# Ced3-han/PepFlowww

Hardware: AMD Instinct MI355X
Metric: residues x denoise-steps / s (higher is better)
Workload: dtype f32 (fp32 storage and accumulation; matrix products as 3 x f16 split MFMA, ~22-bit operands); 1 GPU; cfg4/GPU: B=64 x 128-residue synthetic pockets (112 ctx + 16 gen) per GPU; per_gpu_batch=64, residues=128, global_batch=64, parallelism=batch-shard x1, hipgraph=True, precision=fp32

## Files before the change

pepflowww_amd/csrc/node_track.hip:

```cpp
#include "common.h"
#include "rigid_dev.h"
#include "../../include/pepflow_hip.h"

#ifdef PF_PROFILE
__device__ long long g_prof[64];
#ifndef PF_PROF_LAST
#define PF_PROF_LAST 1
#endif
#define PROF(i) do { if (LAST == (PF_PROF_LAST != 0) && blockIdx.x == 0 && threadIdx.x == 0) g_prof[i] = clock64(); } while (0)
extern "C" int pf_debug_prof(long long* out, int n) {
    return (int)hipMemcpyFromSymbol(out, HIP_SYMBOL(g_prof), sizeof(long long) * n, 0, hipMemcpyDeviceToHost);
}
#else
#define PROF(i)
#endif

namespace {

constexpr int TR = 16;
constexpr int LDX = 132;
constexpr int LDP = 136;
constexpr int NTHR = 512;
#ifndef PF_NT_MINW
#define PF_NT_MINW 2
#endif

struct Planes { _Float16* h; _Float16* l; };

struct LnParams { float g[8], b[8]; };
__device__ __forceinline__ void ln_load(LnParams& p, const float* __restrict__ g, const float* __restrict__ b) {
    const int sub = threadIdx.x & 15;
    const float4 g0 = *reinterpret_cast<const float4*>(g + 8 * sub), g1 = *reinterpret_cast<const float4*>(g + 8 * sub + 4);
    const float4 b0 = *reinterpret_cast<const float4*>(b + 8 * sub), b1 = *reinterpret_cast<const float4*>(b + 8 * sub + 4);
    p.g[0] = g0.x; p.g[1] = g0.y; p.g[2] = g0.z; p.g[3] = g0.w; p.g[4] = g1.x; p.g[5] = g1.y; p.g[6] = g1.z; p.g[7] = g1.w;
    p.b[0] = b0.x; p.b[1] = b0.y; p.b[2] = b0.z; p.b[3] = b0.w; p.b[4] = b1.x; p.b[5] = b1.y; p.b[6] = b1.z; p.b[7] = b1.w;
}
template <int ROWS = 16, bool KFR = false>
__device__ __forceinline__ void ln_tile(float* T, const LnParams& p, float mk, Planes out, int m0, int M, float* gout, _Float16* kf = nullptr, int i0 = 0) {
    const int tid = threadIdx.x;
    if (tid < 16 * ROWS) {
        const int row = tid >> 4, sub = tid & 15, m = m0 + row;
        float v[8];
        {
            const float4 a = *reinterpret_cast<const float4*>(T + row * LDX + 8 * sub);
            const float4 b = *reinterpret_cast<const float4*>(T + row * LDX + 8 * sub + 4);
            v[0] = a.x; v[1] = a.y; v[2] = a.z; v[3] = a.w; v[4] = b.x; v[5] = b.y; v[6] = b.z; v[7] = b.w;
        }
        float s = ((v[0] + v[1]) + (v[2] + v[3])) + ((v[4] + v[5]) + (v[6] + v[7]));
        s = row16_sum(s);
        const float mean = s / 128.f;
        float q = 0.f;
#pragma unroll
        for (int c = 0; c < 8; ++c) { const float d = v[c] - mean; q += d * d; }
        q = row16_sum(q);
        const float rstd = rsqrtf(q / 128.f + 1e-5f);
        float y[8];
#pragma unroll
        for (int c = 0; c < 8; ++c) y[c] = ((v[c] - mean) * rstd * p.g[c] + p.b[c]) * mk;
        *reinterpret_cast<float4*>(T + row * LDX + 8 * sub) = make_float4(y[0], y[1], y[2], y[3]);
        *reinterpret_cast<float4*>(T + row * LDX + 8 * sub + 4) = make_float4(y[4], y[5], y[6], y[7]);
        half4 h0, l0, h1, l1;
        const float y0[4] = {y[0], y[1], y[2], y[3]}, y1[4] = {y[4], y[5], y[6], y[7]};
        split4(y0, h0, l0);
        split4(y1, h1, l1);
        *reinterpret_cast<half4*>(out.h + row * LDP + 8 * sub) = h0;
        *reinterpret_cast<half4*>(out.h + row * LDP + 8 * sub + 4) = h1;
        *reinterpret_cast<half4*>(out.l + row * LDP + 8 * sub) = l0;
        *reinterpret_cast<half4*>(out.l + row * LDP + 8 * sub + 4) = l1;
        if (gout && m < M) {
            *reinterpret_cast<float4*>(gout + (size_t)m * 128 + 8 * sub) = make_float4(y[0], y[1], y[2], y[3]);
            *reinterpret_cast<float4*>(gout + (size_t)m * 128 + 8 * sub + 4) = make_float4(y[4], y[5], y[6], y[7]);
        }
        if constexpr (KFR) {
            if (kf && m < M) {
                pf_kfrag_put(kf, i0 + row, sub >> 1, 2 * (sub & 1), y0);
                pf_kfrag_put(kf, i0 + row, sub >> 1, 2 * (sub & 1) + 1, y1);
            }
        }
    }
}

__device__ __forceinline__ float4 sel4(bool ok, const float4& v) {
    const float f = ok ? 1.f : 0.f;
    return make_float4(v.x * f, v.y * f, v.z * f, v.w * f);
}

__device__ __forceinline__ void put_planes(Planes p, int r, int n, const float (&v)[4]) {
    half4 hi, lo;
    split4(v, hi, lo);
    *reinterpret_cast<half4*>(p.h + r * LDP + n) = hi;
    *reinterpret_cast<half4*>(p.l + r * LDP + n) = lo;
}

template <bool SP, bool DUMP = false, bool PM = false>
__global__ __launch_bounds__(NTHR, PF_NT_MINW) void node_head_kernel(pf_node_head_args a) {
    extern __shared__ __attribute__((aligned(16))) unsigned char smem_raw[];
    constexpr int CK = 256, LDC = CK + 8;
    _Float16* Ch = reinterpret_cast<_Float16*>(smem_raw);
    float* X = reinterpret_cast<float*>(smem_raw + 2 * 2 * TR * LDC * sizeof(_Float16));
    Planes Xa = {reinterpret_cast<_Float16*>(X + TR * LDX), reinterpret_cast<_Float16*>(X + TR * LDX) + TR * LDP};
    const int tid = threadIdx.x, wave = tid >> 6, lane = tid & 63;
    const int r = lane & 15, g = lane >> 4;
    const int m0 = blockIdx.x * TR, M = a.rows;
    if (pf_rows_all_masked(a.key_end, a.key_L, m0, TR, M)) return;
    const int n = wave * 16 + 4 * g;

    constexpr int C0 = PM ? 4 : 0;
    WSplit<1, 8, SP> ws;
    ws.init(a.w_out_f16, 128, PF_IPA_FEATS - C0 * 256, wave * 16);
    ws.prefetch();
    LnParams lnp;
    ln_load(lnp, a.ln_g, a.ln_b);
    const float4 bias_out = *reinterpret_cast<const float4*>(a.b_out + n);
    float4 bias_in[3];
#pragma unroll
    for (int wt = 0; wt < 3; ++wt) bias_in[wt] = *reinterpret_cast<const float4*>(a.b_in + wave * 48 + wt * 16 + 4 * g);
    const int mr = m0 + r;
    const int mrc = mr < M ? mr : M - 1;
    const float rmask_ld = a.mask[mrc];
    const float4 rres_ld = *reinterpret_cast<const float4*>(a.s_in + (size_t)mrc * 128 + n);
    const int srow = tid >> 5, sc4 = tid & 31;
    const bool sok = m0 + srow < M;
    const float* src = a.feats + (size_t)(sok ? m0 + srow : 0) * PF_IPA_FEATS + 4 * sc4;
    constexpr int NCH = PF_IPA_FEATS / CK;
    float4 st[NCH][2];
#pragma unroll
    for (int c = 0; c < NCH; ++c)
#pragma unroll
        for (int hlf = 0; hlf < 2; ++hlf)
            st[c][hlf] = *reinterpret_cast<const float4*>(src + c * CK + hlf * 128);
    auto commit = [&](int c) {
        _Float16* bh = Ch + (c & 1) * 2 * TR * LDC;
        _Float16* bl = bh + TR * LDC;
#pragma unroll
        for (int hlf = 0; hlf < 2; ++hlf) {
            const float4 sv = sel4(sok, st[c][hlf]);
            const float v[4] = {sv.x, sv.y, sv.z, sv.w};
            half4 hi, lo;
            split4(v, hi, lo);
            *reinterpret_cast<half4*>(bh + srow * LDC + hlf * 128 + 4 * sc4) = hi;
            *reinterpret_cast<half4*>(bl + srow * LDC + hlf * 128 + 4 * sc4) = lo;
        }
    };
    if constexpr (PM) {
        auto add4 = [](const float4& p, const float4& q) { return make_float4(p.x + q.x, p.y + q.y, p.z + q.z, p.w + q.w); };
        float4 ev = sel4(sok, st[0][0]), od = sel4(sok, st[0][1]);
#pragma unroll
        for (int c = 1; c < 4; ++c) { ev = add4(ev, sel4(sok, st[c][0])); od = add4(od, sel4(sok, st[c][1])); }
        *reinterpret_cast<float4*>(X + srow * LDX + 4 * sc4) = add4(ev, od);
    }
    commit(C0);
    __syncthreads();
    f32x4 am[1], ac[1];
    acc_zero1<1>(am, ac);
#pragma unroll
    for (int c = C0; c < NCH; ++c) {
        const _Float16* bh = Ch + (c & 1) * 2 * TR * LDC;
        gemm_split16(ws, bh, bh + TR * LDC, LDC, am, ac, (c - C0) * 8, 8);
        if (c + 1 < NCH) commit(c + 1);
        __syncthreads();
    }
    WSplit<3, 4, SP> wq;
    wq.init(a.w_in_f16, 384, 128, wave * 48);
    wq.prefetch();
    {
        const float rmask = rmask_ld * (mr < M ? 1.f : 0.f);
        const float4 rres = sel4(mr < M, rres_ld);
        float4 hs = make_float4(0.f, 0.f, 0.f, 0.f);
        if constexpr (PM) hs = *reinterpret_cast<const float4*>(X + r * LDX + n);
        auto lin = [&](int e, float h) { const float j = join(am[0], ac[0], e); if constexpr (PM) return j + h; else return j; };
        float4 y;
        y.x = (lin(0, hs.x) + bias_out.x) * rmask + rres.x;
        y.y = (lin(1, hs.y) + bias_out.y) * rmask + rres.y;
        y.z = (lin(2, hs.z) + bias_out.z) * rmask + rres.z;
        y.w = (lin(3, hs.w) + bias_out.w) * rmask + rres.w;
        *reinterpret_cast<float4*>(X + r * LDX + n) = y;
        if constexpr (DUMP) { if (mr < M) *reinterpret_cast<float4*>(a.dump_a0 + (size_t)mr * 128 + n) = y; }
    }
    __syncthreads();
    ln_tile(X, lnp, 1.f, Xa, m0, M, a.s_ipa);
    __syncthreads();
    f32x4 qm[3], qc[3];
    acc_zero1<3>(qm, qc);
    gemm_split16(wq, Xa.h, Xa.l, LDP, qm, qc, 0, 4);
    if (mr < M) {
#pragma unroll
        for (int wt = 0; wt < 3; ++wt) {
            float4 y;
            y.x = join(qm[wt], qc[wt], 0) + bias_in[wt].x; y.y = join(qm[wt], qc[wt], 1) + bias_in[wt].y;
            y.z = join(qm[wt], qc[wt], 2) + bias_in[wt].z; y.w = join(qm[wt], qc[wt], 3) + bias_in[wt].w;
            *reinterpret_cast<float4*>(a.qkv + (size_t)mr * 384 + wave * 48 + wt * 16 + 4 * g) = y;
        }
    }
}

constexpr int TR2 = 32;
template <bool SP, bool PM = false>
__global__ __launch_bounds__(NTHR, PF_NT_MINW) void node_head32_kernel(pf_node_head_args a) {
    extern __shared__ __attribute__((aligned(16))) unsigned char smem_raw[];
    constexpr int CK = 256, LDC = CK + 8;
    _Float16* Ch = reinterpret_cast<_Float16*>(smem_raw);
    float* X = reinterpret_cast<float*>(smem_raw + 2 * 2 * TR2 * LDC * sizeof(_Float16));
    Planes Xa = {reinterpret_cast<_Float16*>(X + TR2 * LDX), reinterpret_cast<_Float16*>(X + TR2 * LDX) + TR2 * LDP};
    const int tid = threadIdx.x, wave = tid >> 6, lane = tid & 63;
    const int r = lane & 15, g = lane >> 4;
    int m0 = blockIdx.x * TR2, M = a.rows;
    if (a.key_end) {
        const int tps = (a.key_L + TR2 - 1) / TR2, b = blockIdx.x / tps, i0 = (blockIdx.x - b * tps) * TR2;
        if (i0 >= a.key_end[b]) return;
        m0 = b * a.key_L + i0;
        M = (b + 1) * a.key_L;
    }
    const int n = wave * 16 + 4 * g;

    constexpr int C0 = PM ? 4 : 0;
    WSplit<1, 8, SP> ws;
    ws.init(a.w_out_f16, 128, PF_IPA_FEATS - C0 * 256, wave * 16);
    ws.prefetch();
    LnParams lnp;
    ln_load(lnp, a.ln_g, a.ln_b);
    const float4 bias_out = *reinterpret_cast<const float4*>(a.b_out + n);
    float4 bias_in[3];
#pragma unroll
    for (int wt = 0; wt < 3; ++wt) bias_in[wt] = *reinterpret_cast<const float4*>(a.b_in + wave * 48 + wt * 16 + 4 * g);
    float rmask_ld[2];
    float4 rres_ld[2];
#pragma unroll
    for (int rt = 0; rt < 2; ++rt) {
        const int mr = m0 + rt * 16 + r;
        const int mrc = mr < M ? mr : M - 1;
        rmask_ld[rt] = a.mask[mrc];
        rres_ld[rt] = *reinterpret_cast<const float4*>(a.s_in + (size_t)mrc * 128 + n);
    }
    constexpr int NCH = PF_IPA_FEATS / CK;
    float4 st[2][4];
    auto fetch = [&](int c, float4 (&d)[4]) {
#pragma unroll
        for (int u = 0; u < 4; ++u) {
            const int idx = tid + u * NTHR, row = idx >> 6, c4 = idx & 63;
            const int m = m0 + row < M ? m0 + row : M - 1;
            d[u] = *reinterpret_cast<const float4*>(a.feats + (size_t)m * PF_IPA_FEATS + c * CK + 4 * c4);
        }
    };
    auto commit = [&](int c, const float4 (&d)[4]) {
        _Float16* bh = Ch + (c & 1) * 2 * TR2 * LDC;
        _Float16* bl = bh + TR2 * LDC;
#pragma unroll
        for (int u = 0; u < 4; ++u) {
            const int idx = tid + u * NTHR, row = idx >> 6, c4 = idx & 63;
            const float4 sv = sel4(m0 + row < M, d[u]);
            const float v[4] = {sv.x, sv.y, sv.z, sv.w};
            half4 hi, lo;
            split4(v, hi, lo);
            *reinterpret_cast<half4*>(bh + row * LDC + 4 * c4) = hi;
            *reinterpret_cast<half4*>(bl + row * LDC + 4 * c4) = lo;
        }
    };
    fetch(0, st[0]);
    fetch(1, st[1]);
    if constexpr (PM) {
        auto add4 = [](const float4& p, const float4& q) { return make_float4(p.x + q.x, p.y + q.y, p.z + q.z, p.w + q.w); };
        float4 hsum[4];
#pragma unroll
        for (int c = 0; c < 4; ++c) {
#pragma unroll
            for (int u = 0; u < 4; ++u) {
                const int idx = tid + u * NTHR, row = idx >> 6;
                const float4 v = sel4(m0 + row < M, st[c & 1][u]);
                hsum[u] = c == 0 ? v : add4(hsum[u], v);
            }
            fetch(c + 2, st[c & 1]);
        }
#pragma unroll
        for (int u = 0; u < 4; ++u) {
            const int idx = tid + u * NTHR, row = idx >> 6, c4 = idx & 63;
            float4 o;
            o.x = __shfl_xor(hsum[u].x, 32); o.y = __shfl_xor(hsum[u].y, 32); o.z = __shfl_xor(hsum[u].z, 32); o.w = __shfl_xor(hsum[u].w, 32);
            if (c4 < 32) *reinterpret_cast<float4*>(X + row * LDX + 4 * c4) = add4(hsum[u], o);
        }
    }
    commit(C0, st[C0 & 1]);
    __syncthreads();
    f32x4 am[2][1], ac[2][1];
#pragma unroll
    for (int rt = 0; rt < 2; ++rt) acc_zero1<1>(am[rt], ac[rt]);
#pragma unroll
    for (int c = C0; c < NCH; ++c) {
        if (!PM && c + 2 < NCH) fetch(c + 2, st[c & 1]);
        const _Float16* bh = Ch + (c & 1) * 2 * TR2 * LDC;
        gemm_split16r<1, 8, SP, 2>(ws, bh, bh + TR2 * LDC, LDC, am, ac, (c - C0) * 8, 8);
        if (c + 1 < NCH) commit(c + 1, st[(c + 1) & 1]);
        __syncthreads();
    }
    WSplit<3, 4, SP> wq;
    wq.init(a.w_in_f16, 384, 128, wave * 48);
    wq.prefetch();
#pragma unroll
    for (int rt = 0; rt < 2; ++rt) {
        const int mr = m0 + rt * 16 + r;
        const float rmask = rmask_ld[rt] * (mr < M ? 1.f : 0.f);
        const float4 rres = sel4(mr < M, rres_ld[rt]);
        float4 hs = make_float4(0.f, 0.f, 0.f, 0.f);
        if constexpr (PM) hs = *reinterpret_cast<const float4*>(X + (rt * 16 + r) * LDX + n);
        auto lin = [&](int e, float h) { const float j = join(am[rt][0], ac[rt][0], e); if constexpr (PM) return j + h; else return j; };
        float4 y;
        y.x = (lin(0, hs.x) + bias_out.x) * rmask + rres.x;
        y.y = (lin(1, hs.y) + bias_out.y) * rmask + rres.y;
        y.z = (lin(2, hs.z) + bias_out.z) * rmask + rres.z;
        y.w = (lin(3, hs.w) + bias_out.w) * rmask + rres.w;
        *reinterpret_cast<float4*>(X + (rt * 16 + r) * LDX + n) = y;
    }
    __syncthreads();
    ln_tile<TR2>(X, lnp, 1.f, Xa, m0, M, a.s_ipa);
    __syncthreads();
    f32x4 qm[2][3], qc[2][3];
#pragma unroll
    for (int rt = 0; rt < 2; ++rt) acc_zero1<3>(qm[rt], qc[rt]);
    gemm_split16r<3, 4, SP, 2>(wq, Xa.h, Xa.l, LDP, qm, qc, 0, 4);
#pragma unroll
    for (int rt = 0; rt < 2; ++rt) {
        const int mr = m0 + rt * 16 + r;
        if (mr < M) {
#pragma unroll
            for (int wt = 0; wt < 3; ++wt) {
                float4 y;
                y.x = join(qm[rt][wt], qc[rt][wt], 0) + bias_in[wt].x; y.y = join(qm[rt][wt], qc[rt][wt], 1) + bias_in[wt].y;
                y.z = join(qm[rt][wt], qc[rt][wt], 2) + bias_in[wt].z; y.w = join(qm[rt][wt], qc[rt][wt], 3) + bias_in[wt].w;
                *reinterpret_cast<float4*>(a.qkv + (size_t)mr * 384 + wave * 48 + wt * 16 + 4 * g) = y;
            }
        }
    }
}

template <bool LAST, bool SP, int RT, bool DUMP = false>
__global__ __launch_bounds__(NTHR, PF_NT_MINW) void node_tfmr_kernel(pf_node_tfmr_args a, int LP, int LDS_S) {
    constexpr int TR = 16 * RT;
    extern __shared__ __attribute__((aligned(16))) float smem[];
    float* T0 = smem;
    float* T1 = T0 + TR * LDX;
    float* U = T1 + TR * LDX;
    _Float16* pl = reinterpret_cast<_Float16*>(U + TR * 8);
    Planes Xa = {pl, pl + TR * LDP}, Xb = {pl + 2 * TR * LDP, pl + 3 * TR * LDP};
    float* S = reinterpret_cast<float*>(pl + 4 * TR * LDP);
    const int tid = threadIdx.x, wave = tid >> 6, lane = tid & 63;
    const int r = lane & 15, g = lane >> 4;
    const int L = a.L;
    const int tiles = (L + TR - 1) / TR;
    const int lid = a.key_end ? (int)blockIdx.x : xcd_remap(blockIdx.x, gridDim.x);
    const int b = lid / tiles;
    const int i0 = (lid - b * tiles) * TR;
    const size_t rowb = (size_t)b * L;
    if (a.key_end && i0 >= __builtin_amdgcn_readfirstlane(a.key_end[b])) return;
    if constexpr (LAST) {
        if (a.row_on) {
            int any = 0;
#pragma unroll
            for (int rt = 0; rt < RT; ++rt) any |= a.row_on[((int)rowb + min(i0 + 16 * rt, L - 16)) >> 4];
            if (!__builtin_amdgcn_readfirstlane(any)) return;
        }
    }
    const int m0 = (int)rowb + i0;
    const int M = (int)rowb + L;
    const int n = wave * 16 + 4 * g;
    int mr[RT];
#pragma unroll
    for (int rt = 0; rt < RT; ++rt) mr[rt] = m0 + 16 * rt + r;
    auto dump4 = [&](float* p, int rt, float x, float y, float z, float w) {
        if constexpr (DUMP) { if (mr[rt] < M) *reinterpret_cast<float4*>(p + (size_t)mr[rt] * 128 + n) = make_float4(x, y, z, w); }
    };

    PROF(0);
    const int h = wave & 3;
    float4 q0[RT], q1[RT];
#pragma unroll
    for (int rt = 0; rt < RT; ++rt) {
        const int i = i0 + 16 * rt + r;
        const float* qrow = a.qkv + (rowb + (i < L ? i : 0)) * 384 + h * 32 + 4 * g;
        q0[rt] = *reinterpret_cast<const float4*>(qrow);
        q1[rt] = *reinterpret_cast<const float4*>(qrow + 16);
    }
    const float4 z4 = make_float4(0.f, 0.f, 0.f, 0.f);
    const int par = wave >> 2;
    auto kload = [&](int j0, float4 (&k0)[2], float4 (&k1)[2], float (&km)[2]) {
#pragma unroll
        for (int t = 0; t < 2; ++t) {
            const int j = j0 + 32 * t + r;
            const int jc = j < L ? j : L - 1;
            const float* krow = a.qkv + (rowb + jc) * 384 + 128 + h * 32 + 4 * g;
            k0[t] = *reinterpret_cast<const float4*>(krow);
            k1[t] = *reinterpret_cast<const float4*>(krow + 16);
            km[t] = a.mask[rowb + jc];
        }
    };
    float4 kfA0[2], kfA1[2], kfB0[2], kfB1[2];
    float kfAm[2], kfBm[2];
    kload(16 * par, kfA0, kfA1, kfAm);
    kload(16 * par + 64, kfB0, kfB1, kfBm);
    asm volatile("" ::: "memory");
    const int ct = wave >> 2;
    const float* vcol = a.qkv + rowb * 384 + 256 + h * 32 + ct * 16 + r;
    auto vload = [&](int k0, float (&vb)[4][4]) {
#pragma unroll
        for (int s4 = 0; s4 < 4; ++s4)
#pragma unroll
            for (int t = 0; t < 4; ++t) {
                int j = k0 + 16 * s4 + 4 * g + t;
                j = j < L ? j : L - 1;
                vb[s4][t] = vcol[(size_t)j * 384];
            }
    };
    float vbA[4][4], vbB[4][4];
    vload(0, vbA);
    vload(64, vbB);
    asm volatile("" ::: "memory");
    WSplit<1, 4, SP> ws;
    ws.init(a.w_o_f16, 128, 128, wave * 16);
    ws.prefetch();
    LnParams ln1, ln2, ln3;
    ln_load(ln1, a.n1_g, a.n1_b);
    ln_load(ln2, a.n2_g, a.n2_b);
    if (LAST) ln_load(ln3, a.nt_g, a.nt_b);
    const float4 bias_o = *reinterpret_cast<const float4*>(a.b_o + n), bias_1 = *reinterpret_cast<const float4*>(a.b_1 + n),
                 bias_2 = *reinterpret_cast<const float4*>(a.b_2 + n);
    float4 bias_post = z4, bias_t1 = z4, bias_t2 = z4, bias_t3 = z4, bias_bb = z4, bias_init = z4;
    float4 bias_in[3] = {z4, z4, z4}, bias_pre[4] = {z4, z4, z4, z4};
    float4 rres_ld[RT], rsipa_ld[RT];
#pragma unroll
    for (int rt = 0; rt < RT; ++rt) {
        const int mrc = mr[rt] < M ? mr[rt] : M - 1;
        rres_ld[rt] = *reinterpret_cast<const float4*>(a.resid + (size_t)mrc * 128 + n);
        rsipa_ld[rt] = LAST ? *reinterpret_cast<const float4*>(a.s_ipa + (size_t)mrc * 128 + n) : z4;
    }
    float lnmask_ld = 1.f;
    const int lnrow = m0 + ((tid & (16 * TR - 1)) >> 4);
    auto load_tail_consts = [&]() {
        bias_post = *reinterpret_cast<const float4*>(a.b_post + n);
        bias_t1 = *reinterpret_cast<const float4*>(a.b_t1 + n);
        bias_t2 = *reinterpret_cast<const float4*>(a.b_t2 + n);
        bias_t3 = *reinterpret_cast<const float4*>(a.b_t3 + n);
        bias_bb = *reinterpret_cast<const float4*>(a.b_bb + 4 * (g & 1));
        if (a.has_et) {
            bias_init = *reinterpret_cast<const float4*>(a.b_init + (wave & 3) * 16 + 4 * g);
#pragma unroll
            for (int wt = 0; wt < 4; ++wt) bias_pre[wt] = *reinterpret_cast<const float4*>(a.b_pre + wave * 64 + wt * 16 + 4 * g);
        }
        lnmask_ld = a.mask[lnrow < M ? lnrow : M - 1];
    };
    if (LAST) {
        if (RT == 1) load_tail_consts();
    } else {
#pragma unroll
        for (int wt = 0; wt < 3; ++wt) bias_in[wt] = *reinterpret_cast<const float4*>(a.b_in_next + wave * 48 + wt * 16 + 4 * g);
    }

    PROF(1);
    {
        const float scale = 0.17677669529663687f;
        auto score_block = [&](int j0, const float4 (&k0)[2], const float4 (&k1)[2], const float (&km)[2]) {
#pragma unroll
            for (int t = 0; t < 2; ++t) {
                const int j = j0 + 32 * t + r;
                if (j0 + 32 * t < LP) {
                    const bool keep = j < L && km[t] > 0.5f;
#pragma unroll
                    for (int rt = 0; rt < RT; ++rt) {
                        f32x4 acc = {0.f, 0.f, 0.f, 0.f};
                        acc = mfma16(q0[rt].x, k0[t].x, acc); acc = mfma16(q0[rt].y, k0[t].y, acc); acc = mfma16(q0[rt].z, k0[t].z, acc); acc = mfma16(q0[rt].w, k0[t].w, acc);
                        acc = mfma16(q1[rt].x, k1[t].x, acc); acc = mfma16(q1[rt].y, k1[t].y, acc); acc = mfma16(q1[rt].z, k1[t].z, acc); acc = mfma16(q1[rt].w, k1[t].w, acc);
#pragma unroll
                        for (int e = 0; e < 4; ++e) S[((16 * rt + 4 * g + e) * 4 + h) * LDS_S + j] = keep ? acc[e] * scale : -3.0e38f;
                    }
                }
            }
        };
        score_block(16 * par, kfA0, kfA1, kfAm);
        if (16 * par + 64 < LP) score_block(16 * par + 64, kfB0, kfB1, kfBm);
        for (int j0 = 16 * par + 128; j0 < LP; j0 += 64) {
            float4 kn0[2], kn1[2];
            float knm[2];
            kload(j0, kn0, kn1, knm);
            score_block(j0, kn0, kn1, knm);
        }
    }
    __syncthreads();
    PROF(2);
#pragma unroll
    for (int ps = 0; ps < RT; ++ps) {
        const int sub = lane & 7;
        float* sp = S + ((ps * 8 + wave) * 8 + (lane >> 3)) * LDS_S;
        if (LP <= 256) {
            float4 v[8];
#pragma unroll
            for (int u = 0; u < 8; ++u) {
                const int j = 4 * sub + 32 * u;
                v[u] = j < LP ? *reinterpret_cast<const float4*>(sp + j) : make_float4(-3.0e38f, -3.0e38f, -3.0e38f, -3.0e38f);
            }
            float m = -3.0e38f;
#pragma unroll
            for (int u = 0; u < 8; ++u) m = fmaxf(m, fmaxf(fmaxf(v[u].x, v[u].y), fmaxf(v[u].z, v[u].w)));
            m = fmaxf(m, lane_xor1(m)); m = fmaxf(m, lane_xor2(m)); m = fmaxf(m, lane_xor4(m));
            float sum = 0.f;
#pragma unroll
            for (int u = 0; u < 8; ++u) {
                v[u].x = (v[u].x > -1.0e38f) ? exp_softmax(v[u].x - m) : 0.f; v[u].y = (v[u].y > -1.0e38f) ? exp_softmax(v[u].y - m) : 0.f;
                v[u].z = (v[u].z > -1.0e38f) ? exp_softmax(v[u].z - m) : 0.f; v[u].w = (v[u].w > -1.0e38f) ? exp_softmax(v[u].w - m) : 0.f;
                sum += (v[u].x + v[u].y) + (v[u].z + v[u].w);
            }
            sum += lane_xor1(sum); sum += lane_xor2(sum); sum += lane_xor4(sum);
            const float inv = 1.f / sum;
#pragma unroll
            for (int u = 0; u < 8; ++u) {
                const int j = 4 * sub + 32 * u;
                if (j < LP) *reinterpret_cast<float4*>(sp + j) = make_float4(v[u].x * inv, v[u].y * inv, v[u].z * inv, v[u].w * inv);
            }
        } else {
            float m = -3.0e38f;
            for (int j = sub; j < LP; j += 8) m = fmaxf(m, sp[j]);
            m = fmaxf(m, lane_xor1(m)); m = fmaxf(m, lane_xor2(m)); m = fmaxf(m, lane_xor4(m));
            float sum = 0.f;
            for (int j = sub; j < LP; j += 8) { const float e = (sp[j] > -1.0e38f) ? exp_softmax(sp[j] - m) : 0.f; sp[j] = e; sum += e; }
            sum += lane_xor1(sum); sum += lane_xor2(sum); sum += lane_xor4(sum);
            const float inv = 1.f / sum;
            for (int j = sub; j < LP; j += 8) sp[j] *= inv;
        }
    }
    __syncthreads();
    PROF(3);
    {
        f32x4 acc[RT];
#pragma unroll
        for (int rt = 0; rt < RT; ++rt) acc[rt] = (f32x4){0.f, 0.f, 0.f, 0.f};
        const float* prow = S + (r * 4 + h) * LDS_S + 4 * g;
        auto pv_block = [&](int k0, const float (&vb)[4][4]) {
#pragma unroll
            for (int s4 = 0; s4 < 4; ++s4) {
                if (k0 + 16 * s4 < LP) {
#pragma unroll
                    for (int rt = 0; rt < RT; ++rt) {
                        const float4 pa = *reinterpret_cast<const float4*>(prow + rt * 64 * LDS_S + k0 + 16 * s4);
                        acc[rt] = mfma16(pa.x, vb[s4][0], acc[rt]); acc[rt] = mfma16(pa.y, vb[s4][1], acc[rt]);
                        acc[rt] = mfma16(pa.z, vb[s4][2], acc[rt]); acc[rt] = mfma16(pa.w, vb[s4][3], acc[rt]);
                    }
                }
            }
        };
        pv_block(0, vbA);
        if (64 < LP) pv_block(64, vbB);
        for (int k0 = 128; k0 < LP; k0 += 64) {
            float vn[4][4];
            vload(k0, vn);
            pv_block(k0, vn);
        }
        const int col = h * 32 + ct * 16 + r;
#pragma unroll
        for (int rt = 0; rt < RT; ++rt)
#pragma unroll
            for (int e = 0; e < 4; ++e) {
                const _Float16 hi = (_Float16)acc[rt][e];
                Xa.h[(16 * rt + 4 * g + e) * LDP + col] = hi;
                Xa.l[(16 * rt + 4 * g + e) * LDP + col] = (_Float16)((acc[rt][e] - (float)hi) * PF_LO_SCALE);
                if constexpr (DUMP) { if (m0 + 16 * rt + 4 * g + e < M) a.dump[0][(size_t)(m0 + 16 * rt + 4 * g + e) * 128 + col] = acc[rt][e]; }
            }
    }
    if (LAST && RT == 2) load_tail_consts();
    __syncthreads();
    PROF(4);

    f32x4 am[RT][1], ac[RT][1];
    auto zero = [&]() {
#pragma unroll
        for (int rt = 0; rt < RT; ++rt) acc_zero1<1>(am[rt], ac[rt]);
    };
    auto joined = [&](int rt, const float4& bias, float (&v)[4]) {
        v[0] = join(am[rt][0], ac[rt][0], 0) + bias.x; v[1] = join(am[rt][0], ac[rt][0], 1) + bias.y;
        v[2] = join(am[rt][0], ac[rt][0], 2) + bias.z; v[3] = join(am[rt][0], ac[rt][0], 3) + bias.w;
    };
    auto relu4 = [](float (&v)[4]) {
#pragma unroll
        for (int e = 0; e < 4; ++e) v[e] = fmaxf(v[e], 0.f);
    };
    zero();
    gemm_split16r<1, 4, SP, RT>(ws, Xa.h, Xa.l, LDP, am, ac, 0, 4);
    ws.init(a.w_1_f16, 128, 128, wave * 16);
    ws.prefetch();
#pragma unroll
    for (int rt = 0; rt < RT; ++rt) {
        const float4 rres = sel4(mr[rt] < M, rres_ld[rt]);
        float v[4];
        joined(rt, bias_o, v);
        *reinterpret_cast<float4*>(T1 + (16 * rt + r) * LDX + n) = make_float4(v[0] + rres.x, v[1] + rres.y, v[2] + rres.z, v[3] + rres.w);
        dump4(a.dump[1], rt, v[0] + rres.x, v[1] + rres.y, v[2] + rres.z, v[3] + rres.w);
    }
    __syncthreads();
    ln_tile<TR>(T1, ln1, 1.f, Xb, m0, M, DUMP ? a.dump[2] : nullptr);
    __syncthreads();
    PROF(5);
    zero();
    gemm_split16r<1, 4, SP, RT>(ws, Xb.h, Xb.l, LDP, am, ac, 0, 4);
    ws.init(a.w_2_f16, 128, 128, wave * 16);
    ws.prefetch();
#pragma unroll
    for (int rt = 0; rt < RT; ++rt) {
        float v[4];
        joined(rt, bias_1, v);
        relu4(v);
        put_planes(Xa, 16 * rt + r, n, v);
        dump4(a.dump[3], rt, v[0], v[1], v[2], v[3]);
    }
    __syncthreads();
    PROF(6);
    zero();
    gemm_split16r<1, 4, SP, RT>(ws, Xa.h, Xa.l, LDP, am, ac, 0, 4);
    auto lin2_to_t0 = [&]() {
#pragma unroll
        for (int rt = 0; rt < RT; ++rt) {
            const float4 u = *reinterpret_cast<const float4*>(T1 + (16 * rt + r) * LDX + n);
            float v[4];
            joined(rt, bias_2, v);
            *reinterpret_cast<float4*>(T0 + (16 * rt + r) * LDX + n) = make_float4(v[0] + u.x, v[1] + u.y, v[2] + u.z, v[3] + u.w);
            dump4(a.dump[4], rt, v[0] + u.x, v[1] + u.y, v[2] + u.z, v[3] + u.w);
        }
    };
    if constexpr (!LAST) {
        WSplit<3, 4, SP> wq;
        wq.init(a.w_in_next_f16, 384, 128, wave * 48);
        wq.prefetch();
        lin2_to_t0();
        __syncthreads();
        ln_tile<TR>(T0, ln2, 1.f, Xb, m0, M, a.v_out);
        __syncthreads();
        PROF(7);
        f32x4 qm[RT][3], qc[RT][3];
#pragma unroll
        for (int rt = 0; rt < RT; ++rt) acc_zero1<3>(qm[rt], qc[rt]);
        gemm_split16r<3, 4, SP, RT>(wq, Xb.h, Xb.l, LDP, qm, qc, 0, 4);
#pragma unroll
        for (int rt = 0; rt < RT; ++rt) {
            if (mr[rt] < M) {
#pragma unroll
                for (int wt = 0; wt < 3; ++wt) {
                    float4 y;
                    y.x = join(qm[rt][wt], qc[rt][wt], 0) + bias_in[wt].x; y.y = join(qm[rt][wt], qc[rt][wt], 1) + bias_in[wt].y;
                    y.z = join(qm[rt][wt], qc[rt][wt], 2) + bias_in[wt].z; y.w = join(qm[rt][wt], qc[rt][wt], 3) + bias_in[wt].w;
                    *reinterpret_cast<float4*>(a.qkv_out + (size_t)mr[rt] * 384 + wave * 48 + wt * 16 + 4 * g) = y;
                }
            }
        }
        PROF(8);
    } else {
        ws.init(a.w_post_f16, 128, 128, wave * 16);
        ws.prefetch();
        lin2_to_t0();
        float4 fq = make_float4(1.f, 0.f, 0.f, 0.f);
        float fR[9], fx[3], fmask = 0.f;
        if (tid < TR && m0 + tid < M) {
            const int m = m0 + tid;
            fq = *reinterpret_cast<const float4*>(a.quat_in + (size_t)m * 4);
#pragma unroll
            for (int k = 0; k < 9; ++k) fR[k] = a.rot_in[(size_t)m * 9 + k];
#pragma unroll
            for (int k = 0; k < 3; ++k) fx[k] = a.trans_in[(size_t)m * 3 + k];
            fmask = a.mask[m];
        }
        __syncthreads();
        ln_tile<TR>(T0, ln2, 1.f, Xb, m0, M, DUMP ? a.dump[5] : nullptr);
        __syncthreads();
        PROF(7);
        zero();
        gemm_split16r<1, 4, SP, RT>(ws, Xb.h, Xb.l, LDP, am, ac, 0, 4);
        ws.init(a.w_t1_f16, 128, 128, wave * 16);
        ws.prefetch();
#pragma unroll
        for (int rt = 0; rt < RT; ++rt) {
            const float4 rsipa = sel4(mr[rt] < M, rsipa_ld[rt]);
            float v[4];
            joined(rt, bias_post, v);
            v[0] += rsipa.x; v[1] += rsipa.y; v[2] += rsipa.z; v[3] += rsipa.w;
            *reinterpret_cast<float4*>(T1 + (16 * rt + r) * LDX + n) = make_float4(v[0], v[1], v[2], v[3]);
            put_planes(Xa, 16 * rt + r, n, v);
            dump4(a.dump[6], rt, v[0], v[1], v[2], v[3]);
        }
// ... 182 lines not shown
        if (c4 < 32) {
            const float4 t = *reinterpret_cast<const float4*>(a.node_embed + (size_t)m * 128 + 4 * c4);
            v[0] = t.x; v[1] = t.y; v[2] = t.z; v[3] = t.w;
        } else if (c4 < 64) {
            long long sq = a.seqs[m];
            sq = sq < 0 ? 0 : (sq > 21 ? 21 : sq);
            const float4 t = *reinterpret_cast<const float4*>(a.seq_table + sq * 128 + 4 * (c4 - 32));
            v[0] = t.x; v[1] = t.y; v[2] = t.z; v[3] = t.w;
        } else {
            const float tt = a.t[b] * 2056.f;
#pragma unroll
            for (int e = 0; e < 4; ++e) {
                const int c = 4 * c4 + e;
                float x;
                if (c < 384 && tc_shared) x = TC[b - b_first][c - 256];
                else if (c < 320) x = sinf(tt * a.time_freq[c - 256]);
                else if (c < 384) x = cosf(tt * a.time_freq[c - 320]);
                else if (c < 629) {
                    const int q = c - 384, d = q / 49, k = q - d * 49;
                    const float ang = a.angles[(size_t)m * 5 + d];
                    if (k == 0) x = ang;
                    else if (k < 25) x = sinf(ang * a.ang_freq[k - 1]);
                    else x = cosf(ang * a.ang_freq[k - 25]);
                } else x = 0.f;
                v[e] = x;
            }
        }
        half4 hi, lo;
        split4(v, hi, lo);
        *reinterpret_cast<half4*>(Xf.h + row * LDF + 4 * c4) = hi;
        *reinterpret_cast<half4*>(Xf.l + row * LDF + 4 * c4) = lo;
    }
    if (tid < TR && m0 + tid < M) {
        float R[9], q[4];
#pragma unroll
        for (int k = 0; k < 9; ++k) R[k] = a.rot[(size_t)(m0 + tid) * 9 + k];
        rot_to_quat_dev(R, q);
        *reinterpret_cast<float4*>(a.quat + (size_t)(m0 + tid) * 4) = make_float4(q[0], q[1], q[2], q[3]);
    }
    __syncthreads();
    f32x4 am[1], ac[1];
    acc_zero1<1>(am, ac);
    gemm_split16(w0, Xf.h, Xf.l, LDF, am, ac, 0, 20);
    WSplit<1, 4, SP> w2;
    w2.init(a.w2_f16, 128, 128, wave * 16);
    w2.prefetch();
    {
        const float v[4] = {fmaxf(join(am[0], ac[0], 0) + b0.x, 0.f), fmaxf(join(am[0], ac[0], 1) + b0.y, 0.f),
                            fmaxf(join(am[0], ac[0], 2) + b0.z, 0.f), fmaxf(join(am[0], ac[0], 3) + b0.w, 0.f)};
        put_planes(Xa, r, n, v);
    }
    __syncthreads();
    acc_zero1<1>(am, ac);
    gemm_split16(w2, Xa.h, Xa.l, LDP, am, ac, 0, 4);
    if (mr < M) {
        float4 y;
        y.x = (join(am[0], ac[0], 0) + b2.x) * rmask; y.y = (join(am[0], ac[0], 1) + b2.y) * rmask;
        y.z = (join(am[0], ac[0], 2) + b2.z) * rmask; y.w = (join(am[0], ac[0], 3) + b2.w) * rmask;
        *reinterpret_cast<float4*>(a.s_out + (size_t)mr * 128 + n) = y;
        if (a.k_frag_s) {
            const int b = mr / a.L;
            const float v[4] = {y.x, y.y, y.z, y.w};
            pf_kfrag_put(reinterpret_cast<_Float16*>(a.k_frag_s) + (size_t)b * ((a.L + 15) >> 4) * (PF_KFRAG_TILE_B / 2), mr - b * a.L, wave, g, v);
        }
    }
}

}

extern "C" int pf_input_mixer_fwd(const pf_input_mixer_args* a, pf_stream_t stream) {
    if (!a || !a->node_embed || !a->seq_table || !a->seqs || !a->t || !a->time_freq || !a->ang_freq || !a->angles || !a->w0_f16 ||
        !a->b0 || !a->w2_f16 || !a->b2 || !a->mask || !a->rot || !a->quat || !a->s_out || a->B <= 0 || a->L <= 0)
        return PF_E_BADARG;
    const int rows = a->B * a->L;
    const size_t lds = (size_t)2 * TR * LDF * sizeof(_Float16) + (size_t)2 * TR * LDP * sizeof(_Float16);
    if (a->single_pass) hipLaunchKernelGGL(input_mixer_kernel<true>, dim3((unsigned)((rows + TR - 1) / TR)), dim3(NTHR), lds, (hipStream_t)stream, *a);
    else hipLaunchKernelGGL(input_mixer_kernel<false>, dim3((unsigned)((rows + TR - 1) / TR)), dim3(NTHR), lds, (hipStream_t)stream, *a);
    PF_CHECK_LAUNCH();
    return 0;
}

extern "C" int pf_node_head_fwd(const pf_node_head_args* a, pf_stream_t stream) {
    if (!a || !a->feats || !a->s_in || !a->mask || !a->w_out_f16 || !a->b_out || !a->ln_g || !a->ln_b || !a->w_in_f16 ||
        !a->b_in || !a->s_ipa || !a->qkv || a->rows <= 0)
        return PF_E_BADARG;
    const size_t lds = (size_t)2 * 2 * TR * 264 * sizeof(_Float16) + (size_t)TR * LDX * sizeof(float) +
                       (size_t)2 * TR * LDP * sizeof(_Float16);
    if (a->rows >= pf_cu_count() * TR2 && !a->dump_a0) {
        const size_t lds2 = (size_t)2 * 2 * TR2 * 264 * sizeof(_Float16) + (size_t)TR2 * LDX * sizeof(float) + (size_t)2 * TR2 * LDP * sizeof(_Float16);
        static PfOncePerDevice attr_set;
        if (attr_set.first()) {
            (void)hipFuncSetAttribute((const void*)node_head32_kernel<true>, hipFuncAttributeMaxDynamicSharedMemorySize, 160 * 1024);
            (void)hipFuncSetAttribute((const void*)node_head32_kernel<false>, hipFuncAttributeMaxDynamicSharedMemorySize, 160 * 1024);
            (void)hipFuncSetAttribute((const void*)node_head32_kernel<true, true>, hipFuncAttributeMaxDynamicSharedMemorySize, 160 * 1024);
            (void)hipFuncSetAttribute((const void*)node_head32_kernel<false, true>, hipFuncAttributeMaxDynamicSharedMemorySize, 160 * 1024);
        }
        const bool per_sample = a->key_end && a->key_L > 0 && a->rows % a->key_L == 0;
        pf_node_head_args aa = *a;
        if (!per_sample) aa.key_end = nullptr;
        const dim3 grid(per_sample ? (unsigned)((a->rows / a->key_L) * ((a->key_L + TR2 - 1) / TR2)) : (unsigned)((a->rows + TR2 - 1) / TR2));
        a = &aa;
        if (a->o_premul) {
            if (a->single_pass) hipLaunchKernelGGL((node_head32_kernel<true, true>), grid, dim3(NTHR), lds2, (hipStream_t)stream, *a);
            else hipLaunchKernelGGL((node_head32_kernel<false, true>), grid, dim3(NTHR), lds2, (hipStream_t)stream, *a);
        } else if (a->single_pass) hipLaunchKernelGGL(node_head32_kernel<true>, grid, dim3(NTHR), lds2, (hipStream_t)stream, *a);
        else hipLaunchKernelGGL(node_head32_kernel<false>, grid, dim3(NTHR), lds2, (hipStream_t)stream, *a);
        PF_CHECK_LAUNCH();
        return 0;
    }
    if (a->dump_a0) {
        if (a->single_pass || a->o_premul) return PF_E_BADARG;
        hipLaunchKernelGGL((node_head_kernel<false, true>), dim3((unsigned)((a->rows + TR - 1) / TR)), dim3(NTHR), lds, (hipStream_t)stream, *a);
        PF_CHECK_LAUNCH();
        return 0;
    }
    if (a->o_premul) {
        if (a->single_pass) hipLaunchKernelGGL((node_head_kernel<true, false, true>), dim3((unsigned)((a->rows + TR - 1) / TR)), dim3(NTHR), lds, (hipStream_t)stream, *a);
        else hipLaunchKernelGGL((node_head_kernel<false, false, true>), dim3((unsigned)((a->rows + TR - 1) / TR)), dim3(NTHR), lds, (hipStream_t)stream, *a);
    } else if (a->single_pass) hipLaunchKernelGGL(node_head_kernel<true>, dim3((unsigned)((a->rows + TR - 1) / TR)), dim3(NTHR), lds, (hipStream_t)stream, *a);
    else hipLaunchKernelGGL(node_head_kernel<false>, dim3((unsigned)((a->rows + TR - 1) / TR)), dim3(NTHR), lds, (hipStream_t)stream, *a);
    PF_CHECK_LAUNCH();
    return 0;
}

extern "C" int pf_node_tfmr_fwd(const pf_node_tfmr_args* a, pf_stream_t stream) {
    if (!a || !a->qkv || !a->resid || !a->mask || !a->w_o_f16 || !a->b_o || !a->n1_g || !a->n1_b || !a->w_1_f16 || !a->b_1 ||
        !a->w_2_f16 || !a->b_2 || !a->n2_g || !a->n2_b || a->B <= 0 || a->L <= 0)
        return PF_E_BADARG;
    if (!a->last && (!a->w_in_next_f16 || !a->b_in_next || !a->qkv_out || !a->v_out)) return PF_E_BADARG;
    if (a->last && (!a->s_ipa || !a->w_post_f16 || !a->b_post || !a->w_t1_f16 || !a->b_t1 || !a->w_t2_f16 || !a->b_t2 ||
                    !a->w_t3_f16 || !a->b_t3 || !a->nt_g || !a->nt_b || !a->w_bb_f16 || !a->b_bb || !a->s_out || !a->quat_in ||
                    !a->rot_in || !a->trans_in || !a->quat_out || !a->rot_out || !a->trans_out))
        return PF_E_BADARG;
    if (a->last && a->has_et && (!a->w_init_f16 || !a->b_init || !a->w_pre_f16 || !a->b_pre || !a->pre)) return PF_E_BADARG;
    if (a->last && !a->has_et && a->logits_out) {
        if (!a->ang_out) return PF_E_BADARG;
        for (int net = 0; net < 2; ++net)
            for (int l = 0; l < 3; ++l)
                if (!a->h_w[net][l] || !a->h_b[net][l]) return PF_E_BADARG;
    }
    const int LP = (a->L + 15) / 16 * 16;
    const int LDS_S = LP + 4;
    const int tiles16 = (a->L + 15) / 16;
    auto lds_of = [&](int rt) {
        const int tr = 16 * rt;
        return ((size_t)2 * tr * LDX + tr * 8 + (size_t)tr * 4 * LDS_S) * sizeof(float) + (size_t)4 * tr * LDP * sizeof(_Float16);
    };
    const int RTn = ((long)a->B * tiles16 > pf_cu_count() && a->L > 16 && !a->dump[0] && lds_of(2) <= (size_t)160 * 1024) ? 2 : 1;
    const int TRn = 16 * RTn;
    const size_t lds = lds_of(RTn);
    if (lds > 160 * 1024) return PF_E_TOOLARGE;
    const int tiles = (a->L + TRn - 1) / TRn;
    const dim3 grid((unsigned)(a->B * tiles));
    const int variant = (RTn == 2 ? 4 : 0) + (a->last ? 2 : 0) + (a->single_pass ? 1 : 0);
    static PfOncePerDevice attr_set[8];
#define PF_NT_CASE(V, LASTV, SPV, RTV)                                                                                           \
    case V:                                                                                                                      \
        if (attr_set[V].first()) {                                                                                                      \
            (void)hipFuncSetAttribute((const void*)node_tfmr_kernel<LASTV, SPV, RTV>, hipFuncAttributeMaxDynamicSharedMemorySize, \
                                      160 * 1024);                                                                               \
        }                                                                                                                        \
        hipLaunchKernelGGL((node_tfmr_kernel<LASTV, SPV, RTV>), grid, dim3(NTHR), lds, (hipStream_t)stream, *a, LP, LDS_S);      \
        break;
    if (a->dump[0]) {
        for (int k = 0; k < (a->last ? 11 : 5); ++k)
            if (!a->dump[k]) return PF_E_BADARG;
        if (a->single_pass || RTn != 1) return PF_E_BADARG;
        static PfOncePerDevice dattr[2];
        if (a->last) {
            if (dattr[1].first()) { (void)hipFuncSetAttribute((const void*)node_tfmr_kernel<true, false, 1, true>, hipFuncAttributeMaxDynamicSharedMemorySize, 160 * 1024); }
            hipLaunchKernelGGL((node_tfmr_kernel<true, false, 1, true>), grid, dim3(NTHR), lds, (hipStream_t)stream, *a, LP, LDS_S);
        } else {
            if (dattr[0].first()) { (void)hipFuncSetAttribute((const void*)node_tfmr_kernel<false, false, 1, true>, hipFuncAttributeMaxDynamicSharedMemorySize, 160 * 1024); }
            hipLaunchKernelGGL((node_tfmr_kernel<false, false, 1, true>), grid, dim3(NTHR), lds, (hipStream_t)stream, *a, LP, LDS_S);
        }
        PF_CHECK_LAUNCH();
        return 0;
    }
    switch (variant) {
        PF_NT_CASE(0, false, false, 1) PF_NT_CASE(1, false, true, 1) PF_NT_CASE(2, true, false, 1) PF_NT_CASE(3, true, true, 1)
        PF_NT_CASE(4, false, false, 2) PF_NT_CASE(5, false, true, 2) PF_NT_CASE(6, true, false, 2) PF_NT_CASE(7, true, true, 2)
    }
#undef PF_NT_CASE
    PF_CHECK_LAUNCH();
    return 0;
}
```

Measured before the change: 3.017 million res*step/s.

## Add register-resident attention core for short sequences in node transformer kernel

Adds a REGS variant of the node transformer kernel, used when two 16-row tiles are active and the padded length is at most 128. It loads all K rows and Q into registers and stages V and the mask once in LDS. Scores, softmax and PV then run in registers with cross-lane reductions, so the LDS score matrix round-trip and its two block-wide barriers go away. The trade is much higher register pressure, which may cut occupancy or cause spills. Each wave now handles one head over the full key range, which changes how work is split.

```diff
diff --git a/pepflowww_amd/csrc/node_track.hip b/pepflowww_amd/csrc/node_track.hip
--- a/pepflowww_amd/csrc/node_track.hip
+++ b/pepflowww_amd/csrc/node_track.hip
@@ -1,3 +1,4 @@
+#include <type_traits>
 #include "common.h"
 #include "rigid_dev.h"
 #include "../../include/pepflow_hip.h"
@@ -26,6 +27,15 @@
 #endif
 
 struct Planes { _Float16* h; _Float16* l; };
+
+template <int I, int N, class F> __device__ __forceinline__ void nest_t(int n, F&& f) {
+    if constexpr (I < N) {
+        if (I == 0 || n > I) {
+            f(std::integral_constant<int, I>{});
+            nest_t<I + 1, N>(n, f);
+        }
+    }
+}
 
 struct LnParams { float g[8], b[8]; };
 __device__ __forceinline__ void ln_load(LnParams& p, const float* __restrict__ g, const float* __restrict__ b) {
@@ -332,8 +342,9 @@
     }
 }
 
-template <bool LAST, bool SP, int RT, bool DUMP = false>
+template <bool LAST, bool SP, int RT, bool DUMP = false, bool REGS = false>
 __global__ __launch_bounds__(NTHR, PF_NT_MINW) void node_tfmr_kernel(pf_node_tfmr_args a, int LP, int LDS_S) {
+    static_assert(!REGS || (RT == 2 && !DUMP), "the register core exists for the 32-row inference form only");
     constexpr int TR = 16 * RT;
     extern __shared__ __attribute__((aligned(16))) float smem[];
     float* T0 = smem;
@@ -372,12 +383,35 @@
     PROF(0);
     const int h = wave & 3;
     float4 q0[RT], q1[RT];
-#pragma unroll
-    for (int rt = 0; rt < RT; ++rt) {
-        const int i = i0 + 16 * rt + r;
+    constexpr int MAXKT = 8;
+    const int kt = LP >> 4;
+    float4 rv[MAXKT], rq0 = {}, rq1 = {}, rk0[MAXKT], rk1[MAXKT];
+    float rmk = 0.f;
+    if constexpr (REGS) {
+        const float* vsrc = a.qkv + rowb * 384 + 256 + 4 * (tid & 31);
+#pragma unroll
+        for (int u = 0; u < MAXKT; ++u) rv[u] = *reinterpret_cast<const float4*>(vsrc + (size_t)min(16 * u + (tid >> 5), L - 1) * 384);
+        rmk = a.mask[rowb + min(tid, L - 1)];
+        asm volatile("" ::: "memory");
+        const int i = i0 + 16 * (wave >> 2) + r;
         const float* qrow = a.qkv + (rowb + (i < L ? i : 0)) * 384 + h * 32 + 4 * g;
-        q0[rt] = *reinterpret_cast<const float4*>(qrow);
-        q1[rt] = *reinterpret_cast<const float4*>(qrow + 16);
+        rq0 = *reinterpret_cast<const float4*>(qrow);
+        rq1 = *reinterpret_cast<const float4*>(qrow + 16);
+#pragma unroll
+        for (int t = 0; t < MAXKT; ++t) {
+            const float* krow = a.qkv + (rowb + min(16 * t + r, L - 1)) * 384 + 128 + h * 32 + 4 * g;
+            rk0[t] = *reinterpret_cast<const float4*>(krow);
+            rk1[t] = *reinterpret_cast<const float4*>(krow + 16);
+        }
+        asm volatile("" ::: "memory");
+    } else {
+#pragma unroll
+        for (int rt = 0; rt < RT; ++rt) {
+            const int i = i0 + 16 * rt + r;
+            const float* qrow = a.qkv + (rowb + (i < L ? i : 0)) * 384 + h * 32 + 4 * g;
+            q0[rt] = *reinterpret_cast<const float4*>(qrow);
+            q1[rt] = *reinterpret_cast<const float4*>(qrow + 16);
+        }
     }
     const float4 z4 = make_float4(0.f, 0.f, 0.f, 0.f);
     const int par = wave >> 2;
@@ -394,9 +428,11 @@
     };
     float4 kfA0[2], kfA1[2], kfB0[2], kfB1[2];
     float kfAm[2], kfBm[2];
-    kload(16 * par, kfA0, kfA1, kfAm);
-    kload(16 * par + 64, kfB0, kfB1, kfBm);
-    asm volatile("" ::: "memory");
+    if constexpr (!REGS) {
+        kload(16 * par, kfA0, kfA1, kfAm);
+        kload(16 * par + 64, kfB0, kfB1, kfBm);
+        asm volatile("" ::: "memory");
+    }
     const int ct = wave >> 2;
     const float* vcol = a.qkv + rowb * 384 + 256 + h * 32 + ct * 16 + r;
     auto vload = [&](int k0, float (&vb)[4][4]) {
@@ -410,9 +446,11 @@
             }
     };
     float vbA[4][4], vbB[4][4];
-    vload(0, vbA);
-    vload(64, vbB);
-    asm volatile("" ::: "memory");
+    if constexpr (!REGS) {
+        vload(0, vbA);
+        vload(64, vbB);
+        asm volatile("" ::: "memory");
+    }
     WSplit<1, 4, SP> ws;
     ws.init(a.w_o_f16, 128, 128, wave * 16);
     ws.prefetch();
@@ -454,7 +492,68 @@
     }
 
     PROF(1);
-    {
+    if constexpr (REGS) {
+        float* Vs = S;
+        nest_t<0, MAXKT>(kt, [&](auto iu) __attribute__((always_inline)) {
+            constexpr int u = decltype(iu)::value;
+            *reinterpret_cast<float4*>(Vs + (16 * u + (tid >> 5)) * LDX + 4 * (tid & 31)) = make_float4(rv[u].x, rv[u].y, rv[u].z, rv[u].w);
+        });
+        if (tid < LP) Vs[(tid & ~3) * LDX + 128 + (tid & 3)] = tid < L ? rmk : 0.f;
+        lds_barrier();
+        const float scale = 0.17677669529663687f;
+        float4 sc[MAXKT];
+#pragma unroll
+        for (int t = 0; t < MAXKT; ++t) sc[t] = make_float4(-3.0e38f, -3.0e38f, -3.0e38f, -3.0e38f);
+        nest_t<0, MAXKT>(kt, [&](auto it) __attribute__((always_inline)) {
+            constexpr int t = decltype(it)::value;
+            const float4 km = *reinterpret_cast<const float4*>(Vs + (16 * t + 4 * g) * LDX + 128);
+            f32x4 acc = {0.f, 0.f, 0.f, 0.f};
+            acc = mfma16(rk0[t].x, rq0.x, acc); acc = mfma16(rk0[t].y, rq0.y, acc); acc = mfma16(rk0[t].z, rq0.z, acc); acc = mfma16(rk0[t].w, rq0.w, acc);
+            acc = mfma16(rk1[t].x, rq1.x, acc); acc = mfma16(rk1[t].y, rq1.y, acc); acc = mfma16(rk1[t].z, rq1.z, acc); acc = mfma16(rk1[t].w, rq1.w, acc);
+            sc[t].x = km.x > 0.5f ? acc[0] * scale : -3.0e38f; sc[t].y = km.y > 0.5f ? acc[1] * scale : -3.0e38f;
+            sc[t].z = km.z > 0.5f ? acc[2] * scale : -3.0e38f; sc[t].w = km.w > 0.5f ? acc[3] * scale : -3.0e38f;
+        });
+        PROF(2);
+        float m = -3.0e38f;
+#pragma unroll
+        for (int t = 0; t < MAXKT; ++t) m = fmaxf(m, fmaxf(fmaxf(sc[t].x, sc[t].y), fmaxf(sc[t].z, sc[t].w)));
+        m = max_xor32(max_xor16(m));
+        float sum2[2] = {0.f, 0.f};
+#pragma unroll
+        for (int t = 0; t < MAXKT; ++t) {
+            sc[t].x = (sc[t].x > -1.0e38f) ? exp_softmax(sc[t].x - m) : 0.f; sc[t].y = (sc[t].y > -1.0e38f) ? exp_softmax(sc[t].y - m) : 0.f;
+            sc[t].z = (sc[t].z > -1.0e38f) ? exp_softmax(sc[t].z - m) : 0.f; sc[t].w = (sc[t].w > -1.0e38f) ? exp_softmax(sc[t].w - m) : 0.f;
+            sum2[t & 1] += (sc[t].x + sc[t].y) + (sc[t].z + sc[t].w);
+        }
+        const float sum = sum_xor32(sum_xor16(sum2[0])) + sum_xor32(sum_xor16(sum2[1]));
+        const float inv = 1.f / sum;
+#pragma unroll
+        for (int t = 0; t < MAXKT; ++t) { sc[t].x *= inv; sc[t].y *= inv; sc[t].z *= inv; sc[t].w *= inv; }
+        PROF(3);
+        f32x4 o[2] = {{0.f, 0.f, 0.f, 0.f}, {0.f, 0.f, 0.f, 0.f}};
+        const float* vb = Vs + 4 * g * LDX + 32 * h + r;
+        nest_t<0, MAXKT>(kt, [&](auto it) __attribute__((always_inline)) {
+            constexpr int t = decltype(it)::value;
+#pragma unroll
+            for (int c = 0; c < 2; ++c) {
+                const float* vt = vb + 16 * t * LDX + 16 * c;
+                o[c] = mfma16(sc[t].x, vt[0], o[c]); o[c] = mfma16(sc[t].y, vt[LDX], o[c]);
+                o[c] = mfma16(sc[t].z, vt[2 * LDX], o[c]); o[c] = mfma16(sc[t].w, vt[3 * LDX], o[c]);
+            }
+        });
+        const int rt = wave >> 2;
+#pragma unroll
+        for (int c = 0; c < 2; ++c) {
+            const int col = h * 32 + c * 16 + r;
+#pragma unroll
+            for (int e = 0; e < 4; ++e) {
+                const _Float16 hi = (_Float16)o[c][e];
+                Xa.h[(16 * rt + 4 * g + e) * LDP + col] = hi;
+                Xa.l[(16 * rt + 4 * g + e) * LDP + col] = (_Float16)((o[c][e] - (float)hi) * PF_LO_SCALE);
+            }
+        }
+    }
+    if constexpr (!REGS) {
         const float scale = 0.17677669529663687f;
         auto score_block = [&](int j0, const float4 (&k0)[2], const float4 (&k1)[2], const float (&km)[2]) {
 #pragma unroll
@@ -482,10 +581,12 @@
             score_block(j0, kn0, kn1, knm);
         }
     }
-    __syncthreads();
-    PROF(2);
-#pragma unroll
-    for (int ps = 0; ps < RT; ++ps) {
+    if constexpr (!REGS) {
+        __syncthreads();
+        PROF(2);
+    }
+#pragma unroll
+    for (int ps = 0; ps < (REGS ? 0 : RT); ++ps) {
         const int sub = lane & 7;
         float* sp = S + ((ps * 8 + wave) * 8 + (lane >> 3)) * LDS_S;
         if (LP <= 256) {
@@ -524,9 +625,11 @@
             for (int j = sub; j < LP; j += 8) sp[j] *= inv;
         }
     }
-    __syncthreads();
-    PROF(3);
-    {
+    if constexpr (!REGS) {
+        __syncthreads();
+        PROF(3);
+    }
+    if constexpr (!REGS) {
         f32x4 acc[RT];
 #pragma unroll
         for (int rt = 0; rt < RT; ++rt) acc[rt] = (f32x4){0.f, 0.f, 0.f, 0.f};
@@ -1015,15 +1118,17 @@
     if (lds > 160 * 1024) return PF_E_TOOLARGE;
     const int tiles = (a->L + TRn - 1) / TRn;
     const dim3 grid((unsigned)(a->B * tiles));
-    const int variant = (RTn == 2 ? 4 : 0) + (a->last ? 2 : 0) + (a->single_pass ? 1 : 0);
-    static PfOncePerDevice attr_set[8];
-#define PF_NT_CASE(V, LASTV, SPV, RTV)                                                                                           \
+    const bool regs = RTn == 2 && LP <= 128;
+    const int variant = (regs ? 8 : 0) + (RTn == 2 ? 4 : 0) + (a->last ? 2 : 0) + (a->single_pass ? 1 : 0);
+    static PfOncePerDevice attr_set[16];
+#define PF_NT_CASE(V, LASTV, SPV, RTV, REGSV)                                                                                    \
     case V:                                                                                                                      \
-        if (attr_set[V].first()) {                                                                                                      \
-            (void)hipFuncSetAttribute((const void*)node_tfmr_kernel<LASTV, SPV, RTV>, hipFuncAttributeMaxDynamicSharedMemorySize, \
-                                      160 * 1024);                                                                               \
+        if (attr_set[V].first()) {                                                                                               \
+            (void)hipFuncSetAttribute((const void*)node_tfmr_kernel<LASTV, SPV, RTV, false, REGSV>,                              \
+                                      hipFuncAttributeMaxDynamicSharedMemorySize, 160 * 1024);                                   \
         }                                                                                                                        \
-        hipLaunchKernelGGL((node_tfmr_kernel<LASTV, SPV, RTV>), grid, dim3(NTHR), lds, (hipStream_t)stream, *a, LP, LDS_S);      \
+        hipLaunchKernelGGL((node_tfmr_kernel<LASTV, SPV, RTV, false, REGSV>), grid, dim3(NTHR), lds, (hipStream_t)stream, *a, LP, \
+                           LDS_S);                                                                                               \
         break;
     if (a->dump[0]) {
         for (int k = 0; k < (a->last ? 11 : 5); ++k)
@@ -1041,8 +1146,9 @@
         return 0;
     }
     switch (variant) {
-        PF_NT_CASE(0, false, false, 1) PF_NT_CASE(1, false, true, 1) PF_NT_CASE(2, true, false, 1) PF_NT_CASE(3, true, true, 1)
-        PF_NT_CASE(4, false, false, 2) PF_NT_CASE(5, false, true, 2) PF_NT_CASE(6, true, false, 2) PF_NT_CASE(7, true, true, 2)
+        PF_NT_CASE(0, false, false, 1, false) PF_NT_CASE(1, false, true, 1, false) PF_NT_CASE(2, true, false, 1, false) PF_NT_CASE(3, true, true, 1, false)
+        PF_NT_CASE(4, false, false, 2, false) PF_NT_CASE(5, false, true, 2, false) PF_NT_CASE(6, true, false, 2, false) PF_NT_CASE(7, true, true, 2, false)
+        PF_NT_CASE(12, false, false, 2, true) PF_NT_CASE(13, false, true, 2, true) PF_NT_CASE(14, true, false, 2, true) PF_NT_CASE(15, true, true, 2, true)
     }
 #undef PF_NT_CASE
     PF_CHECK_LAUNCH();
```

Result: no change. 3.026 million res*step/s, median of 6 (+0.3%).
